# EveryVoiceTTS/FastSpeech2_lightning

Measured on AMD Instinct MI355X. Metric: mel-frames/sec (train fwd+bwd+optimizer, whole job), higher is better.
Workload: dtype f32

## Files before the change

### fastspeech2_lightning_amd/csrc/gemm_ws32.hip

```cpp
#include "gemm2_core.h"

namespace {

constexpr int W32_THREADS = 512, W32_KT = 8;
constexpr int W32_TILE_FLOATS = W32_KT * 32 * 32;
#ifndef W32_TWO_CHAINS
#define W32_TWO_CHAINS 0
#endif

template <int EPI, bool TWO>
__global__ __launch_bounds__(W32_THREADS) void gemmws32_kernel(GemmP p, int n_slices, int n_streams, int n_row_tiles) {
  __shared__ __attribute__((aligned(16))) float lds[2 * W32_TILE_FLOATS];
  const Fs2GemmArgs& a = p.a;
  const int tid = threadIdx.x, lane = tid & 63, l31 = lane & 31, h = lane >> 5;
  const int wave = __builtin_amdgcn_readfirstlane(tid >> 6);
  const int bx = blockIdx.x & 7, bj = blockIdx.x >> 3;
  const int slice = bj % n_slices;
  const int stream = (bj / n_slices) * 8 + bx;
  const int ns0 = slice * 256, nw0 = ns0 + wave * 32;
  const int cnt = stream < n_row_tiles ? (n_row_tiles - 1 - stream) / n_streams + 1 : 0;

  f32x4 wf[32];
  {
    const float* wrow = a.B + (long long)(nw0 + l31) * a.ldb + 4 * h;
    const bool ok = nw0 + l31 < a.Nc;
#pragma unroll
    for (int q = 0; q < 32; ++q) wf[q] = ok ? *reinterpret_cast<const f32x4*>(wrow + 8 * q) : f32x4{0.f, 0.f, 0.f, 0.f};
  }

  const __amdgpu_buffer_rsrc_t ra = __builtin_amdgcn_make_buffer_rsrc((void*)a.A, 0, a.Mc * a.lda * 4, 0x00020000);
  const int avoff = (((tid >> 3) & 31) * a.lda + (tid >> 8) * 32 + (((tid & 7) ^ ((tid >> 4) & 7)) << 2)) * 4;
  const int tile_stride = 32 * a.lda * 4;
  auto dma = [&](int k) {
    if (k >= cnt) return;
    const int soff = (stream + k * n_streams) * tile_stride;
    float* dst = lds + (k & 1) * W32_TILE_FLOATS;
#pragma unroll
    for (int it = 0; it < 4; ++it) blds16(ra, avoff, soff + 256 * it, dst + (it * W32_THREADS + wave * 64) * 4);
  };
  const unsigned lds0 = (unsigned)(unsigned long long)(__attribute__((address_space(3))) float*)lds;
  unsigned ard[4];
#pragma unroll
  for (int g = 0; g < 4; ++g) ard[g] = lds0 + (l31 * 32 + (((2 * g + h) ^ ((l31 >> 1) & 7)) << 2)) * 4;

  f32x16 acc[1][1];
  constexpr int STORES = TWO ? 32 : 16;
  float* C = a.C;
  const bool late = wave >= 4;
  dma(0);
  for (int i = 0; i < cnt; ++i) {
    if (i == 0 || (late && i == 1)) wait_vmcnt_barrier<0>(); else wait_vmcnt_barrier<STORES>();
    dma(i + 1);
    if (late && i > 0)
      gemm_epilogue_impl<64, 64, EPI>(p, acc, C, a.ldc, (stream + (i - 1) * n_streams) * 32, ns0, 0, wave, lane);
    const unsigned sb = (i & 1) * (W32_TILE_FLOATS * 4);
    f32x16 acc2;
#pragma unroll
    for (int r = 0; r < 16; ++r) acc[0][0][r] = acc2[r] = 0.f;
    f32x4 af[3];
#define W32_RD(Q_) lds_rd128<((Q_) >> 2) * 4096>(af[(Q_) % 3], ard[(Q_) & 3] + sb);
#define W32_MM(Q_, PENDING)                                                                                        \
  lds_wait<PENDING>();                                                                                             \
  pin(af[(Q_) % 3]);                                                                                               \
  _Pragma("unroll") for (int j = 0; j < 4; ++j) {                                                                  \
    if (W32_TWO_CHAINS && (j & 1))                                                                                 \
      acc2 = __builtin_amdgcn_mfma_f32_32x32x2f32(af[(Q_) % 3][j], wf[Q_][j], acc2, 0, 0, 0);                       \
    else                                                                                                           \
      acc[0][0] = __builtin_amdgcn_mfma_f32_32x32x2f32(af[(Q_) % 3][j], wf[Q_][j], acc[0][0], 0, 0, 0);            \
  }
#define W32_STEP(Q_) W32_RD((Q_) + 2) W32_MM(Q_, 2)
    W32_RD(0) W32_RD(1)
    W32_STEP(0) W32_STEP(1) W32_STEP(2) W32_STEP(3) W32_STEP(4) W32_STEP(5) W32_STEP(6) W32_STEP(7)
    W32_STEP(8) W32_STEP(9) W32_STEP(10) W32_STEP(11) W32_STEP(12) W32_STEP(13) W32_STEP(14) W32_STEP(15)
    W32_STEP(16) W32_STEP(17) W32_STEP(18) W32_STEP(19) W32_STEP(20) W32_STEP(21) W32_STEP(22) W32_STEP(23)
    W32_STEP(24) W32_STEP(25) W32_STEP(26) W32_STEP(27) W32_STEP(28) W32_STEP(29)
    W32_MM(30, 1) W32_MM(31, 0)
#undef W32_STEP
#undef W32_RD
#undef W32_MM
    if (W32_TWO_CHAINS) {
#pragma unroll
      for (int r = 0; r < 16; ++r) acc[0][0][r] += acc2[r];
    }
    if (!late) gemm_epilogue_impl<64, 64, EPI>(p, acc, C, a.ldc, (stream + i * n_streams) * 32, ns0, 0, wave, lane);
  }
  if (late && cnt > 0)
    gemm_epilogue_impl<64, 64, EPI>(p, acc, C, a.ldc, (stream + (cnt - 1) * n_streams) * 32, ns0, 0, wave, lane);
  asm volatile("s_waitcnt vmcnt(0)" ::: "memory");
}

template <int EPI>
int go32(GemmP& p, dim3 grid, int n_slices, int n_streams, int n_row_tiles, hipStream_t s) {
  if (p.a.out_pre) gemmws32_kernel<EPI, true><<<grid, dim3(W32_THREADS), 0, s>>>(p, n_slices, n_streams, n_row_tiles);
  else gemmws32_kernel<EPI, false><<<grid, dim3(W32_THREADS), 0, s>>>(p, n_slices, n_streams, n_row_tiles);
  FS2_LAUNCH_CHECK();
  return 0;
}

}

int fs2_gemmws32_launch(GemmP& p, hipStream_t s) {
  const Fs2GemmArgs& a = p.a;
  if (a.operand_bf16 != 0 || !a.a_kcontig || !a.b_kcontig || a.taps != 1 || a.splitk != 1 || a.R != 256 || a.colsum)
    return FS2HIP_EINVAL;
  if ((a.ldb % 4) || ((uintptr_t)a.B % 16) || a.epi < FS2_EPI_STORE || a.epi > FS2_EPI_DACT) return FS2HIP_EINVAL;
  if (a.out_pre && a.epi != FS2_EPI_ACT) return FS2HIP_EINVAL;
  if ((long long)(a.Mc + 64) * a.lda * 4 >= 0x7fffffffLL) return FS2HIP_EINVAL;
  static int n_cu = 0;
  if (n_cu == 0) {
    int dev = 0;
    hipDeviceProp_t prop;
    if (hipGetDevice(&dev) != hipSuccess || hipGetDeviceProperties(&prop, dev) != hipSuccess) return FS2HIP_EINVAL;
    n_cu = prop.multiProcessorCount;
  }
  const int n_slices = (a.Nc + 255) / 256;
  const int per_xcd = n_cu / 8;
  if (per_xcd < 1 || n_slices > per_xcd) return FS2HIP_EINVAL;
  const int n_row_tiles = (a.Mc + 31) / 32;
  int streams_per_xcd = per_xcd / n_slices;
  while (streams_per_xcd > 1 && (streams_per_xcd - 1) * 8 >= n_row_tiles) --streams_per_xcd;
  const int n_streams = streams_per_xcd * 8;
  dim3 grid(8 * streams_per_xcd * n_slices);
  switch (a.epi) {
    case FS2_EPI_ACT: return go32<FS2_EPI_ACT>(p, grid, n_slices, n_streams, n_row_tiles, s);
    case FS2_EPI_RESID: return go32<FS2_EPI_RESID>(p, grid, n_slices, n_streams, n_row_tiles, s);
    case FS2_EPI_DACT: return go32<FS2_EPI_DACT>(p, grid, n_slices, n_streams, n_row_tiles, s);
    default: return go32<0>(p, grid, n_slices, n_streams, n_row_tiles, s);
  }
}
```

Before: 950,800.

## Specialize DMA to late waves and add a dedicated per-wave GEMM epilogue

By default only the four late waves issue the LDS-bound buffer loads (each doing twice as many), and the early waves use a plain barrier instead of waiting on vmcnt. This lets early waves run MFMA and their stores without waiting on outstanding store counts. The shared epilogue is replaced with a specialized per-wave epilogue struct. It precomputes buffer resources, offsets, bias and dropout state once, then uses buffer loads and stores. It also adds optional timestamp instrumentation and an extra launch-time bounds check for the epilogue buffers. The risks are load imbalance across waves and correctness subtleties in the new barrier and vmcnt scheme.

```diff
diff --git a/fastspeech2_lightning_amd/csrc/gemm_ws32.hip b/fastspeech2_lightning_amd/csrc/gemm_ws32.hip
--- a/fastspeech2_lightning_amd/csrc/gemm_ws32.hip
+++ b/fastspeech2_lightning_amd/csrc/gemm_ws32.hip
@@ -7,6 +7,148 @@
 #ifndef W32_TWO_CHAINS
 #define W32_TWO_CHAINS 0
 #endif
+
+#ifdef W32_STAMPS
+constexpr int W32_ST_WAIT = 0, W32_ST_DMA = 1, W32_ST_MFMA = 2, W32_ST_EPI = 3, W32_ST_PROLOGUE = 4, W32_ST_DRAIN = 5;
+constexpr int W32_STAMP_BLOCKS = 1024;
+__device__ long long w32_stamps[W32_STAMP_BLOCKS * 8 * 8];
+#define W32_STAMP_DECL long long st_prev = __builtin_amdgcn_s_memtime(), st_sum[6] = {0, 0, 0, 0, 0, 0}
+#define W32_STAMP(i)                                       \
+  {                                                        \
+    const long long st_now = __builtin_amdgcn_s_memtime(); \
+    st_sum[i] += st_now - st_prev;                         \
+    st_prev = st_now;                                      \
+  }
+#define W32_STAMP_FLUSH(wave_, lane_, cnt_)                                          \
+  if ((lane_) == 0 && blockIdx.x < W32_STAMP_BLOCKS) {                               \
+    long long* o_ = w32_stamps + ((long long)blockIdx.x * 8 + (wave_)) * 8;          \
+    for (int i_ = 0; i_ < 6; ++i_) o_[i_] += st_sum[i_];                             \
+    o_[6] += (cnt_);                                                                 \
+    o_[7] += 1;                                                                      \
+  }
+#define W32_STAMP_SETTLE() asm volatile("s_waitcnt vmcnt(0)" ::: "memory")
+#else
+#define W32_STAMP_DECL
+#define W32_STAMP(i)
+#define W32_STAMP_FLUSH(wave_, lane_, cnt_)
+#define W32_STAMP_SETTLE()
+#endif
+#ifndef W32_DMA_ALL_WAVES
+#define W32_DMA_ALL_WAVES 0
+#endif
+#ifndef W32_SHARED_EPILOGUE
+#define W32_SHARED_EPILOGUE 0
+#endif
+
+template <int EPI, bool TWO>
+struct W32Epi {
+  __amdgpu_buffer_rsrc_t rc, rx;
+  int vc, vx;
+  int ldc4, ldx4;
+  float bias;
+  Fs2Drop drop;
+  unsigned hv;
+  unsigned sh, thresh;
+  float scale;
+  bool par;
+
+  __device__ __forceinline__ void setup(const GemmP& p, int n, int h, int lane) {
+    const Fs2GemmArgs& a = p.a;
+    const bool col = n < a.Nc;
+    rc = fs2_epi_rsrc(a.C, a.Mc, a.ldc);
+    ldc4 = a.ldc * 4;
+    vc = col ? (4 * h * a.ldc + n) * 4 : FS2_EPI_OOB;
+    bias = (a.bias && col) ? a.bias[n] : 0.f;
+    const float* x = EPI == FS2_EPI_ACT ? a.out_pre : EPI == FS2_EPI_RESID ? a.resid : EPI == FS2_EPI_DACT ? a.aux : nullptr;
+    const int ldx = EPI == FS2_EPI_ACT ? a.ldpre : EPI == FS2_EPI_RESID ? a.ldr : EPI == FS2_EPI_DACT ? a.ldaux : 0;
+    rx = fs2_epi_rsrc(x, a.Mc, ldx);
+    ldx4 = ldx * 4;
+    vx = col ? (4 * h * ldx + n) * 4 : FS2_EPI_OOB;
+    drop = fs2_resolve_drop(p.drop);
+    thresh = drop.thresh;
+    scale = drop.scale;
+    asm volatile("" : "+v"(thresh), "+v"(scale));
+    par = lane & 1;
+    sh = (unsigned)par << 4;
+    hv = (unsigned)(4 * h * a.ldc + n);
+    if ((a.ldc & 1) == 0) hv = (hv + (par ? (unsigned)a.ldc : 0u)) >> 1;
+  }
+
+  __device__ __forceinline__ void run(const Fs2GemmArgs& a, const f32x16& acc, int m0) const {
+    int sc[16], sx[16];
+    {
+      int c = m0 * ldc4, x = m0 * ldx4;
+      const int c5 = 5 * ldc4, x5 = 5 * ldx4;
+#pragma unroll
+      for (int r = 0; r < 16; ++r) {
+        asm volatile("" : "+s"(c), "+s"(x));
+        sc[r] = c;
+        sx[r] = x;
+        c += (r & 3) == 3 ? c5 : ldc4;
+        x += (r & 3) == 3 ? x5 : ldx4;
+      }
+    }
+    float v[16], xin[16];
+    if (EPI == FS2_EPI_RESID || EPI == FS2_EPI_DACT) {
+#pragma unroll
+      for (int r = 0; r < 16; ++r) xin[r] = fs2_buf_load(rx, vx, sx[r]);
+    }
+#pragma unroll
+    for (int r = 0; r < 16; ++r) v[r] = a.alpha * acc[r] + bias;
+    if (EPI == FS2_EPI_ACT) {
+      if (TWO) {
+#pragma unroll
+        for (int r = 0; r < 16; ++r) fs2_buf_store(rx, vx, sx[r], v[r]);
+      }
+      if (a.act == FS2_ACT_RELU) {
+#pragma unroll
+        for (int r = 0; r < 16; ++r) v[r] = fs2_act(FS2_ACT_RELU, v[r]);
+      } else if (a.act == FS2_ACT_SILU) {
+#pragma unroll
+        for (int r = 0; r < 16; ++r) v[r] = fs2_act(FS2_ACT_SILU, v[r]);
+      } else if (a.act == FS2_ACT_TANH) {
+#pragma unroll
+        for (int r = 0; r < 16; ++r) v[r] = fs2_act(FS2_ACT_TANH, v[r]);
+      }
+    } else if (EPI == FS2_EPI_DACT) {
+      if (a.act == FS2_ACT_RELU) {
+#pragma unroll
+        for (int r = 0; r < 16; ++r) v[r] *= fs2_dact(FS2_ACT_RELU, xin[r]);
+      } else if (a.act == FS2_ACT_SILU) {
+#pragma unroll
+        for (int r = 0; r < 16; ++r) v[r] *= fs2_dact(FS2_ACT_SILU, xin[r]);
+      } else if (a.act == FS2_ACT_TANH) {
+#pragma unroll
+        for (int r = 0; r < 16; ++r) v[r] *= fs2_dact(FS2_ACT_TANH, xin[r]);
+      }
+    }
+    if (EPI > 0 && drop.on) {
+      if ((a.ldc & 1) == 0) {
+#pragma unroll
+        for (int r = 0; r < 16; r += 2) {
+          const uint32_t H = fs2_hash32_lo(drop.seed, hv + ((unsigned)sc[r] >> 3));
+          const uint32_t Hn = (uint32_t)__builtin_amdgcn_mov_dpp((int)H, 0xB1, 0xF, 0xF, true);
+          const uint32_t ha = par ? Hn : H, hb = par ? H : Hn;
+          v[r] *= ((ha >> sh) & 0xffffu) < thresh ? 0.f : scale;
+          v[r + 1] *= ((hb >> sh) & 0xffffu) < thresh ? 0.f : scale;
+        }
+      } else {
+#pragma unroll
+        for (int r = 0; r < 16; ++r) {
+          const unsigned idx = hv + ((unsigned)sc[r] >> 2);
+          const uint32_t hh = fs2_hash32_lo(drop.seed, idx >> 1);
+          v[r] *= ((idx & 1) ? (hh >> 16) : (hh & 0xffffu)) < thresh ? 0.f : scale;
+        }
+      }
+    }
+    if (EPI == FS2_EPI_RESID) {
+#pragma unroll
+      for (int r = 0; r < 16; ++r) v[r] = xin[r] + a.res_scale * v[r];
+    }
+#pragma unroll
+    for (int r = 0; r < 16; ++r) fs2_buf_store(rc, vc, sc[r], v[r]);
+  }
+};
 
 template <int EPI, bool TWO>
 __global__ __launch_bounds__(W32_THREADS) void gemmws32_kernel(GemmP p, int n_slices, int n_streams, int n_row_tiles) {
@@ -19,6 +161,30 @@
   const int stream = (bj / n_slices) * 8 + bx;
   const int ns0 = slice * 256, nw0 = ns0 + wave * 32;
   const int cnt = stream < n_row_tiles ? (n_row_tiles - 1 - stream) / n_streams + 1 : 0;
+  const bool late = wave >= 4;
+  W32_STAMP_DECL;
+
+  const __amdgpu_buffer_rsrc_t ra = __builtin_amdgcn_make_buffer_rsrc((void*)a.A, 0, a.Mc * a.lda * 4, 0x00020000);
+  const int dw = W32_DMA_ALL_WAVES ? wave : wave & 3;
+  const int dt = dw * 64 + lane;
+  const int avoff = (((dt >> 3) & 31) * a.lda + (dt >> 8) * 32 + (((dt & 7) ^ ((dt >> 4) & 7)) << 2)) * 4;
+  const int tile_stride = 32 * a.lda * 4;
+  auto dma = [&](int k) {
+    if (k >= cnt) return;
+    const int soff = (stream + k * n_streams) * tile_stride;
+    float* dst = lds + (k & 1) * W32_TILE_FLOATS + dw * 256;
+    if (W32_DMA_ALL_WAVES) {
+#pragma unroll
+      for (int it = 0; it < 4; ++it) blds16(ra, avoff, soff + 256 * it, dst + it * 2048);
+    } else if (late) {
+#pragma unroll
+      for (int it = 0; it < 4; ++it) {
+        blds16(ra, avoff, soff + 256 * it, dst + it * 2048);
+        blds16(ra, avoff, soff + 256 * it + 128, dst + it * 2048 + 1024);
+      }
+    }
+  };
+  if (!W32_DMA_ALL_WAVES) dma(0);
 
   f32x4 wf[32];
   {
@@ -27,17 +193,7 @@
 #pragma unroll
     for (int q = 0; q < 32; ++q) wf[q] = ok ? *reinterpret_cast<const f32x4*>(wrow + 8 * q) : f32x4{0.f, 0.f, 0.f, 0.f};
   }
-
-  const __amdgpu_buffer_rsrc_t ra = __builtin_amdgcn_make_buffer_rsrc((void*)a.A, 0, a.Mc * a.lda * 4, 0x00020000);
-  const int avoff = (((tid >> 3) & 31) * a.lda + (tid >> 8) * 32 + (((tid & 7) ^ ((tid >> 4) & 7)) << 2)) * 4;
-  const int tile_stride = 32 * a.lda * 4;
-  auto dma = [&](int k) {
-    if (k >= cnt) return;
-    const int soff = (stream + k * n_streams) * tile_stride;
-    float* dst = lds + (k & 1) * W32_TILE_FLOATS;
-#pragma unroll
-    for (int it = 0; it < 4; ++it) blds16(ra, avoff, soff + 256 * it, dst + (it * W32_THREADS + wave * 64) * 4);
-  };
+  if (W32_DMA_ALL_WAVES) dma(0);
   const unsigned lds0 = (unsigned)(unsigned long long)(__attribute__((address_space(3))) float*)lds;
   unsigned ard[4];
 #pragma unroll
@@ -45,14 +201,29 @@
 
   f32x16 acc[1][1];
   constexpr int STORES = TWO ? 32 : 16;
+#if W32_SHARED_EPILOGUE
   float* C = a.C;
-  const bool late = wave >= 4;
-  dma(0);
+#define W32_EPILOGUE(M0_) gemm_epilogue_impl<64, 64, EPI>(p, acc, C, a.ldc, (M0_), ns0, 0, wave, lane)
+#else
+  W32Epi<EPI, TWO> epi;
+  epi.setup(p, nw0 + l31, h, lane);
+#define W32_EPILOGUE(M0_) epi.run(a, acc[0][0], (M0_))
+#endif
+  W32_STAMP_SETTLE();
+  W32_STAMP(W32_ST_PROLOGUE)
   for (int i = 0; i < cnt; ++i) {
-    if (i == 0 || (late && i == 1)) wait_vmcnt_barrier<0>(); else wait_vmcnt_barrier<STORES>();
+    if (late || W32_DMA_ALL_WAVES) {
+      if (i == 0 || (late && i == 1)) wait_vmcnt_barrier<0>(); else wait_vmcnt_barrier<STORES>();
+    } else {
+      __builtin_amdgcn_s_barrier();
+    }
+    W32_STAMP(W32_ST_WAIT)
     dma(i + 1);
-    if (late && i > 0)
-      gemm_epilogue_impl<64, 64, EPI>(p, acc, C, a.ldc, (stream + (i - 1) * n_streams) * 32, ns0, 0, wave, lane);
+    W32_STAMP(W32_ST_DMA)
+    if (late && i > 0) {
+      W32_EPILOGUE((stream + (i - 1) * n_streams) * 32);
+      W32_STAMP(W32_ST_EPI)
+    }
     const unsigned sb = (i & 1) * (W32_TILE_FLOATS * 4);
     f32x16 acc2;
 #pragma unroll
@@ -82,11 +253,20 @@
 #pragma unroll
       for (int r = 0; r < 16; ++r) acc[0][0][r] += acc2[r];
     }
-    if (!late) gemm_epilogue_impl<64, 64, EPI>(p, acc, C, a.ldc, (stream + i * n_streams) * 32, ns0, 0, wave, lane);
-  }
-  if (late && cnt > 0)
-    gemm_epilogue_impl<64, 64, EPI>(p, acc, C, a.ldc, (stream + (cnt - 1) * n_streams) * 32, ns0, 0, wave, lane);
+#ifdef W32_STAMPS
+    asm volatile("" : "+v"(acc[0][0]));
+#endif
+    W32_STAMP(W32_ST_MFMA)
+    if (!late) {
+      W32_EPILOGUE((stream + i * n_streams) * 32);
+      W32_STAMP(W32_ST_EPI)
+    }
+  }
+  if (late && cnt > 0) W32_EPILOGUE((stream + (cnt - 1) * n_streams) * 32);
+#undef W32_EPILOGUE
   asm volatile("s_waitcnt vmcnt(0)" ::: "memory");
+  W32_STAMP(W32_ST_DRAIN)
+  W32_STAMP_FLUSH(wave, lane, cnt)
 }
 
 template <int EPI>
@@ -106,6 +286,8 @@
   if ((a.ldb % 4) || ((uintptr_t)a.B % 16) || a.epi < FS2_EPI_STORE || a.epi > FS2_EPI_DACT) return FS2HIP_EINVAL;
   if (a.out_pre && a.epi != FS2_EPI_ACT) return FS2HIP_EINVAL;
   if ((long long)(a.Mc + 64) * a.lda * 4 >= 0x7fffffffLL) return FS2HIP_EINVAL;
+  const int ldx = a.epi == FS2_EPI_ACT ? (a.out_pre ? a.ldpre : 0) : a.epi == FS2_EPI_RESID ? a.ldr : a.epi == FS2_EPI_DACT ? a.ldaux : 0;
+  if ((long long)(a.Mc + 64) * (a.ldc > ldx ? a.ldc : ldx) * 4 >= 0x7fffffffLL) return FS2HIP_EINVAL;
   static int n_cu = 0;
   if (n_cu == 0) {
     int dev = 0;
```

Measured after the change: 947,900. About the same (-0.3%).
